# xindonglin99/allsteps_isaaclab

Measured on AMD Instinct MI355X. Metric: env-steps/sec (whole node), Allsteps-v0 at 4096 envs, 1/2/4/8 MI355X, higher is better.
Workload: dtype f32; 1 GPU; Allsteps-v0 biped walker, 4096 envs/GPU, stone curriculum level 0, decimation 4 x dt 1/240; num_envs_per_gpu=4096, global_envs=4096, parallelism=dp1 (env shards, no collective in step)

## Files before the change

allsteps_isaaclab_amd/csrc/allsteps_kernels.hip:

```cpp
#include <hip/hip_runtime.h>

#include "../../include/allsteps.h"
#include "allsteps_device.h"
#include "allsteps_kernels.h"

#include "step_scratch.h"
#include "step_lanes.h"
#include "step_dynamics.h"
#include "step_collide.h"
#include "step_solve.h"
#include "step_report.h"
#include "step_task.h"

namespace as {

template <int NV, uint64_t SKIP>
__global__ __launch_bounds__(kStepThreads) __attribute__((amdgpu_waves_per_eu(2, 2))) void k_step(StepArgs P) {
  __shared__ Smem sm;
  CK* Kc = (CK*)P.consts;
  const Consts& K = *(const Consts*)Kc;
  const int el = threadIdx.x >> 5, lane = threadIdx.x & 31;
  const int n = P.n;
  EnvS& s = sm.env[el];
  const as_state_t& st = P.st;
  Stamp ts{P.stamps, sm.stamp_acc, 0ull};
  ts.start();
  int e_raw = xcd_block(blockIdx.x, gridDim.x) * EPB + el;
  if (P.wave_map) e_raw = P.wave_map[EPB * blockIdx.x + el];
  const ConstV4* rowp = (const ConstV4*)&Kc->lane[lane];
  u32x4 rc[kLaneChunks];
#pragma unroll
  for (int k = 0; k < kLaneChunks; ++k) rc[k] = rowp[k];
  const int cur = *(const __attribute__((address_space(4))) int32_t*)st.curriculum;
  const float cur_gain = Kc->task.gain_curriculum[lane < 10 ? lane : 0];
  const float cur_term = Kc->task.term_curriculum[lane < 10 ? lane : 0];
  const bool valid = e_raw < n;
  const int e = valid ? e_raw : n - 1;
  if (P.wave_map && blockIdx.x >= (gridDim.x >> 1)) __builtin_amdgcn_s_setprio(1);
  const __attribute__((address_space(4))) as_model_t& m = Kc->model;
  const int nh = m.num_hinges;
  const __attribute__((address_space(4))) as_task_t& T = Kc->task;
  const int l3 = lane < 3 ? lane : 0, l4 = lane < 4 ? lane : 0, lh = lane < nh ? lane : 0;
  const int ns3 = 3 * T.num_steps;
  const int k0 = lane < ns3 ? lane : 0, k1 = lane + G < ns3 ? lane + G : 0;
  const float v_rp = st.root_pos[l3 * n + e], v_rl = st.root_lin[l3 * n + e], v_ra = st.root_ang[l3 * n + e];
  const float v_rq = st.root_quat[l4 * n + e];
  const float v_q = st.q[lh * n + e], v_qd = st.qd[lh * n + e];
  const float* actp = P.mode != kModeReset ? P.actions : st.q;
// ... 49 lines not shown
  if (lane < 4) s.root_quat[lane] = v_rq;
  if (lane == 0) { s.ndrop = 0; s.nrows = 0; }
  if (lane < nh) {
    int i = (int)rc[9].w - 1;
    s.qi[i] = v_q;
    s.u[6 + i] = v_qd;
    float a = fminf(fmaxf(v_a, -1.f), 1.f);
    s.act[lane] = a;
    s.tau[i] = gain * row_gear * a;
    s.qt[i] = Kc->act.action_scale * a + row_dq;
    if (P.cmd) {
      s.tau[i] = v_c;
      s.qt[i] = v_c;
    }
  }
  if (lane < ns3) s.stones[lane] = v_s0;
  if (lane + G < ns3) s.stones[lane + G] = v_s1;
  if (lane < kPkWords) s.pk[lane] = v_pk;
  __syncthreads();
  ts.mark(kStLoad);
  const bool do_physics = P.mode == kModeStep || P.mode == kModePhysics;
  if (do_physics) {
    const int substeps = Kc->sim.substeps;
    for (int left = substeps - 1; left >= 0; --left) {
      const ReportDesc* rp = P.rep;
      asm volatile("" : "+s"(rp));
      if (rp && left == 0) report_store_qd(rp, n, Kc, s, lane, e, valid);
      substep<NV, SKIP>(K, sm, s, lane, tp, gc, lc, mask, ts);
      rp = P.rep;
      asm volatile("" : "+s"(rp));
      if (rp) report_store(rp, n, s, lane, e, valid, left);
    }
  }
  const u32x4* rowg = (const u32x4*)&K.lane[lane];
  const u32x4 rr8 = rowg[8], rr9 = rowg[9];
  const float rs_q = __uint_as_float(rr8.z), rs_qm = __uint_as_float(rr8.w), rs_sg = __uint_as_float(rr9.x);
  const float rs_lo = __uint_as_float(rr9.y), rs_hi = __uint_as_float(rr9.z);
  const int rs_li = (int)rr9.w;
  float rd_m = 0.f, rd_n = 0.f;
  if (P.reset_draws && P.mode != kModePhysics) {
    rd_m = P.reset_draws[(size_t)e * 22];
    rd_n = P.reset_draws[(size_t)e * 22 + 1 + lh];
  }
  asm volatile("" ::: "memory");
  if (do_physics) {
    fk<false>(*Kc, s, lane, tp, lc, Kc->max_path);
    if (lane == 0) { s.mask[0] = mask[0]; s.mask[1] = mask[1]; s.mask[2] = mask[2]; s.mask[3] = mask[3]; }
  }
  ts.mark(kStFKFinal);
  if (lane == 0 && !do_physics) { s.mask[0] = mask[0]; s.mask[1] = mask[1]; }
  __syncthreads();
  float bp[9];
  if (do_physics) {
    const int ls[3] = {m.torso_link, m.foot_link[0], m.foot_link[1]};
    for (int b = 0; b < 3; ++b)
      for (int k = 0; k < 3; ++k) bp[3 * b + k] = s.root_pos[k] + s.p[ls[b]][k];
  } else {
    for (int k = 0; k < 9; ++k) bp[k] = __uint_as_float(s.pk[kPkBody + k]);
  }
  int idx = (int)s.pk[kPkIdx], prev = (int)s.pk[kPkPrev], next = (int)s.pk[kPkNext], count = (int)s.pk[kPkCount];
  int swing = (int)s.pk[kPkSwing], ep_len = (int)s.pk[kPkEpLen];
  float pot = __uint_as_float(s.pk[kPkPot]), old_pot = __uint_as_float(s.pk[kPkOldPot]);
  float fc[2] = {__uint_as_float(s.pk[kPkFc0]), __uint_as_float(s.pk[kPkFc1])};
  uint32_t episode = s.pk[kPkEpisode];
  bool done = false;
  Useful u{};
  if (P.mode == kModeStep || P.mode == kModeTask) {
    ep_len += 1;
    compute_useful(T, s.root_pos, s.root_quat, bp, s.stones, 1, s.mask[0], s.mask[1], idx, prev, next, count,
                   swing, pot, old_pot, fc, true, u);
    float a2 = 0.f, en = 0.f;
    int atlim = 0;
    if (lane < nh) {
      const int li = rs_li;
      float a = s.act[lane];
      a2 = a * a;
      en = fabsf(s.u[6 + li - 1] * a);
      atlim = fabsf(scale_transform(s.qi[li - 1], rs_lo, rs_hi)) > 0.99f;
    }
    a2 = half_sum(a2);
    en = half_sum(en);
    uint64_t bl = __ballot(atlim != 0);
    int nlim = __popcll(bl >> (32 * el) & 0xffffffffull);
    const float* lv = s.u;
    float speed = sqrtf(lv[0] * lv[0] + lv[1] * lv[1] + lv[2] * lv[2]);
    bool time_out = ep_len >= T.max_episode_length - 1;
    bool fell = u.h < term_h;
    bool so_fast = speed > 5.0f;
    bool died = s.root_pos[2] < T.fall_abs;
    bool terminated = fell || so_fast || died;
// ... 1 lines not shown
    bool roll_v = (u.roll > 0.4f) || (u.roll < -0.4f);
    bool pitch_v = (u.pitch > 0.4f) || (u.pitch < -0.2f);
    float roll_cost = roll_v ? fabsf(u.roll) : 0.f;
    float pitch_cost = pitch_v ? fabsf(u.pitch) : 0.f;
    float speed_cost = speed > 1.6f ? speed - 1.6f : 0.f;
    float action_cost = T.action * sqrtf(a2);
    float energy_cost = T.energy * en;
    float limit_cost = (float)nlim * T.joint_limit;
    bool cond = u.reached && count == 1 && idx < T.num_steps - 1;
    float step_rew = cond ? 50.0f * as_expf(-u.dist_s / 0.25f) : 0.f;
    bool bonus_c = idx == T.num_steps - 1 && u.body_dist < 0.15f;
    float total = T.alive + progress;
    total = total - roll_cost;
    total = total - pitch_cost;
    total = total - speed_cost;
    total = total - energy_cost;
    total = total - action_cost;
    total = total - limit_cost;
    total = total + step_rew;
    total = total + (bonus_c ? 10.0f : 0.f);
    float rew = terminated ? T.death : total;
    done = terminated || time_out;
    if (valid && lane == 0) {
      P.reward[e] = rew;
      P.terminated[e] = terminated ? 1 : 0;
      P.truncated[e] = time_out ? 1 : 0;
    }
  } else if (P.mode == kModeReset) {
    done = P.reset_mask == nullptr || P.reset_mask[e] != 0;
  }
  if (P.mode != kModePhysics) {
    const int cidx = valid ? idx : 0;
    const bool vdone = valid && done;
    const int wsum = __builtin_amdgcn_readlane(cidx, 0) + __builtin_amdgcn_readlane(cidx, 32);
    const bool wdone = __any(vdone);
    const int ndr = valid ? s.ndrop : 0;
    const int wdrop = __builtin_amdgcn_readlane(ndr, 0) + __builtin_amdgcn_readlane(ndr, 32);
    if (threadIdx.x == 0) {
      atomicAdd(&P.counters[kCntStride * (1 + (int)(blockIdx.x % kCntSlots))], wsum);
      if (wdrop) atomicAdd(&P.counters[kCntDropped], wdrop);
      if (wdone) P.counters[0] = 1;
      if (T.regen_footsteps) P.counters[kCntLevel] = cur;
    }
  }
  ts.mark(kStTask);
  const bool any_done = __any(done);
  const bool regen = T.regen_footsteps && P.mode != kModePhysics && done && idx > T.num_steps / 2;
  if (P.mode != kModePhysics && any_done) {
    if (done) {
      float dm = rd_m, dn = rd_n;
      if (!P.reset_draws) {
        float blk[4];
        philox_block(P.seed, (uint32_t)(P.env_offset + e), episode, 0u, kResetTag, blk);
        dm = blk[0];
        if (lane < nh) {
          const int k = 1 + lane;
          philox_block(P.seed, (uint32_t)(P.env_offset + e), episode, (uint32_t)(k >> 2), kResetTag, blk);
          const int sl = k & 3;
          dn = sl == 0 ? blk[0] : (sl == 1 ? blk[1] : (sl == 2 ? blk[2] : blk[3]));
        }
      }
      ep_len = 0;
      old_pot = 0.f; pot = 0.f; count = 0; swing = 0; idx = 1; prev = 0; next = 2;
      const bool mirror = dm > 0.5f;
      if (mirror) swing ^= 1;
      if (lane < nh) {
        const float sign = mirror ? rs_sg : 1.f;
        float jp = mirror ? rs_qm : rs_q;
        float jv = 0.f * sign;
        int li = rs_li;
        float x = jp + (dn * (T.noise_hi - T.noise_lo) + T.noise_lo);
        float sc = fminf(fmaxf(scale_transform(x, rs_lo, rs_hi), T.clip_lo), T.clip_hi);
        s.qi[li - 1] = unscale_transform(sc, rs_lo, rs_hi);
        s.u[6 + li - 1] = jv;
      }
      if (lane < 3) {
        const float ir[3] = {T.init_root[0], T.init_root[1], T.init_root[2]};
        s.root_pos[lane] = lane == 0 ? ir[0] : (lane == 1 ? ir[1] : ir[2]);
        s.u[lane] = 0.f;
        s.u[3 + lane] = 0.f;
      }
      if (lane == 0) {
        float sg = mirror ? -1.f : 1.f;
        s.root_quat[0] = 1.f;
        s.root_quat[1] = 0.f * sg;
        s.root_quat[2] = 0.f * sg;
        s.root_quat[3] = 0.f * sg;
      }
      episode += 1u;
    }
    __syncthreads();
    fk<false>(*Kc, s, lane, tp, lc, Kc->max_path);
    if (done) {
      const int ls[3] = {m.torso_link, m.foot_link[0], m.foot_link[1]};
      for (int b = 0; b < 3; ++b)
        for (int k = 0; k < 3; ++k) bp[3 * b + k] = s.root_pos[k] + s.p[ls[b]][k];
    }
  }
  __syncthreads();
  if (P.obs) {
    int i2 = idx, p2 = prev, n2 = next, c2 = count, w2 = swing;
    float pot2 = pot, op2 = old_pot, fc2[2] = {fc[0], fc[1]};
    Useful u2 = u;
    compute_useful(T, s.root_pos, s.root_quat, bp, s.stones, 1, s.mask[0], s.mask[1], i2, p2, n2, c2, w2, pot2,
                   op2, fc2, true, u2, any_done || !(P.mode == kModeStep || P.mode == kModeTask));
    float* ob = s.x.obs;
    uint32_t* side = P.side;
    if (lane == 0) {
      ob[0] = u2.h;
      ob[1] = u2.roll;
      ob[2] = u2.pitch;
      float vb[3];
      quat_rotate_inverse(s.root_quat, s.u, vb);
      ob[3] = vb[0]; ob[4] = vb[1]; ob[5] = vb[2];
      ob[48] = fc2[0];
      ob[49] = fc2[1];
    }
    if (lane < nh) {
      const int li = rs_li;
      ob[6 + lane] = scale_transform(s.qi[li - 1], rs_lo, rs_hi);
      ob[27 + lane] = fminf(fmaxf(s.u[6 + li - 1] * T.dof_vel_scale, -5.f), 5.f);
    }
    if (lane < 6) {
      const int t = lane < 3 ? lane : lane - 3;
      const int ti = lane < 3 ? (t == 0 ? p2 : (t == 1 ? i2 : n2)) : (t == 0 ? prev : (t == 1 ? idx : next));
      const float tw[3] = {s.stones[3 * ti], s.stones[3 * ti + 1], s.stones[3 * ti + 2]};
      float o3[3];
      subtract_frame_transforms(s.root_pos, s.root_quat, tw, o3);
      if (lane < 3) {
        for (int k = 0; k < 3; ++k) ob[50 + 3 * t + k] = o3[k];
      } else if (valid) {
        for (int k = 0; k < 3; ++k) side[(kSideState + 2 + 3 * t + k) * n + e] = __float_as_uint(o3[k]);
      }
    }
    __syncthreads();
    if (valid) {
      float* orow = P.obs + (size_t)e * AS_OBS_DIM;
      orow[lane] = ob[lane];
      if (lane < AS_OBS_DIM - 32) orow[32 + lane] = ob[32 + lane];
      if (lane == 0) {
        const uint32_t sv[kSideState + 2] = {(uint32_t)idx, (uint32_t)prev, (uint32_t)next, (uint32_t)count,
                                             (uint32_t)swing, __float_as_uint(pot), __float_as_uint(old_pot),
                                             __float_as_uint(fc[0]), __float_as_uint(fc[1]),
                                             __float_as_uint(fc[0]), __float_as_uint(fc[1])};
        for (int k = 0; k < kSideState + 2; ++k) side[k * n + e] = sv[k];
        side[kSideRegen * n + e] = regen ? 1u : 0u;
      }
    }
    idx = i2; prev = p2; next = n2; count = c2; swing = w2;
    pot = pot2; old_pot = op2; fc[0] = fc2[0]; fc[1] = fc2[1];
  }
  ts.mark(kStReset);
  if (valid) {
    if (lane < 3) {
      st.root_pos[lane * n + e] = s.root_pos[lane];
      st.root_lin[lane * n + e] = s.u[lane];
      st.root_ang[lane * n + e] = s.u[3 + lane];
    }
    if (lane < 4) st.root_quat[lane * n + e] = s.root_quat[lane];
    if (lane < nh) {
      int i = rs_li - 1;
      st.q[lane * n + e] = s.qi[i];
      st.qd[lane * n + e] = s.u[6 + i];
    }
    if (lane < 9) {
      float v = bp[0];
#pragma unroll
      for (int k = 1; k < 9; ++k) v = (lane == k) ? bp[k] : v;
      st.body_pos[lane * n + e] = v;
    }
    if (lane == 0) {
      P.side[kSideCost * n + e] = done ? 0u : (uint32_t)s.nrows;
      st.contact_mask[e] = s.mask[0];
      st.contact_mask[n + e] = s.mask[1];
      if (st.contact_mask_hind) {
        st.contact_mask_hind[e] = s.mask[2];
        st.contact_mask_hind[n + e] = s.mask[3];
      }
      if (P.mode != kModePhysics) {
        st.idx[e] = idx; st.prev[e] = prev; st.next[e] = next; st.count[e] = count; st.swing[e] = swing;
        st.ep_len[e] = ep_len; st.pot[e] = pot; st.old_pot[e] = old_pot;
        st.foot_contact[e] = fc[0]; st.foot_contact[n + e] = fc[1];
        st.episode[e] = episode;
      }
    }
  }
  ts.mark(kStStore);
  ts.flush();
}

}

#include "task_kernels.h"
#include "body_state_kernel.h"
#include "contact_forces_kernel.h"
#include "noise_kernels.h"
#include "event_kernels.h"
#include "contact_timer_kernels.h"
#include "ray_caster_kernels.h"
#include "imu_kernels.h"
#include "frame_transformer_kernels.h"
#include "ray_camera_kernels.h"
#include "command_kernels.h"
#include "observation_kernels.h"
#include "reward_kernels.h"
#include "termination_kernels.h"
#include "action_kernels.h"

namespace as {


bool step_supported_nv(int nv) { return nv == 27 || nv == 18; }

hipError_t launch_step(const StepArgs& a, int nv, bool sweep_skip, hipStream_t stream) {
  int blocks = (a.n + EPB - 1) / EPB;
  if (nv == 27 && sweep_skip)
    hipLaunchKernelGGL((k_step<27, kSweepSkip27>), dim3(blocks), dim3(kStepThreads), 0, stream, a);
  else if (nv == 27)
    hipLaunchKernelGGL((k_step<27, 0ull>), dim3(blocks), dim3(kStepThreads), 0, stream, a);
  else if (nv == 18 && sweep_skip)
    hipLaunchKernelGGL((k_step<18, kSweepSkip18>), dim3(blocks), dim3(kStepThreads), 0, stream, a);
  else if (nv == 18)
    hipLaunchKernelGGL((k_step<18, 0ull>), dim3(blocks), dim3(kStepThreads), 0, stream, a);
  else
    return hipErrorInvalidValue;
  return hipGetLastError();
}

hipError_t launch_obs(const ObsArgs& a, hipStream_t stream) {
  int blocks = (a.n + 63) / 64;
  hipLaunchKernelGGL(k_obs, dim3(blocks), dim3(64), 0, stream, a);
  return hipGetLastError();
}

hipError_t launch_stones(const StonesArgs& a, hipStream_t stream) {
  int blocks = (a.n + 255) / 256;
  hipLaunchKernelGGL(k_stones, dim3(blocks), dim3(256), 0, stream, a);
  return hipGetLastError();
}

hipError_t launch_quad(const QuadArgs& a, hipStream_t stream) {
  hipLaunchKernelGGL(k_quad<false>, dim3((a.n + kQuadEnvs - 1) / kQuadEnvs), dim3(4 * kQuadEnvs), 0, stream, a,
                     (const uint8_t*)nullptr);
  return hipGetLastError();
}

// ... 148 lines not shown
```

allsteps_isaaclab_amd/csrc/step_collide.h:

```cpp
#pragma once

#include <hip/hip_runtime.h>

#include "allsteps_pair_group.h"
#include "step_lanes.h"
#include "step_scratch.h"

namespace as {


__device__ void emit_contact(EnvS& s, int slot, int ncap, int link, int link2, int stone, int foot, const float* P,
                             const float* n, float sep, float r) {
  if (slot >= ncap) return;
  s.clink[slot] = link; s.clink2[slot] = link2; s.cstone[slot] = stone; s.cfoot[slot] = foot; s.csep[slot] = sep;
  for (int k = 0; k < 3; ++k) { s.cn[slot][k] = n[k]; s.cpt[slot][k] = P[k] - n[k] * r; }
}

struct GeomC {
  int link, type, foot;
  float r, p0[3], p1[3];
  uint32_t anc;
};
__device__ __forceinline__ float capsule_contact_sel(const float* a1, const float* b1, float r1, const float* a2,
                                                     const float* b2, float r2, float* P, float* n) {
// ... 16 lines not shown
  const float sq = as_clamp01((hi ? b - c : -c) / a);
  const float s = pa ? 0.f : (pe || lo || hi) ? sq : sm;
  const float t = pa ? (pe ? 0.f : as_clamp01(tq)) : pe ? 0.f : lo ? 0.f : hi ? 1.f : tq;
  float c1[3], c2[3], w[3];
#pragma unroll
  for (int k = 0; k < 3; ++k) {
    c1[k] = fmaf(s, d1[k], a1[k]);
    c2[k] = fmaf(t, d2[k], a2[k]);
    w[k] = c1[k] - c2[k];
  }
  const float dist = sqrtf(as_dot3(w, w));
  const bool nz = dist > 1e-9f;
  const float inv = 1.0f / dist;
  n[0] = nz ? w[0] * inv : 0.f;
  n[1] = nz ? w[1] * inv : 0.f;
  n[2] = nz ? w[2] * inv : 1.f;
  const float sep = dist - r1 - r2;
  const float off = fmaf(0.5f, sep, r2);
#pragma unroll
  for (int k = 0; k < 3; ++k) P[k] = fmaf(off, n[k], c2[k]);
  return sep;
}

__device__ __forceinline__ int collide(const Consts& K, EnvS& s, int lane, int ncap, const GeomC& gc, const float* h,
                                       float margin, int gcap, Stamp& ts) {
  const as_model_t& m = K.model;
  const int nst = K.task.num_steps, ng = m.num_geoms, npri = m.num_priority_geoms, nsp = m.num_self_pairs;
  constexpr int kSelfW = AS_MAX_SELF_PAIRS / G;
  int spw[kSelfW];
#pragma unroll
  for (int i = 0; i < kSelfW; ++i) spw[i] = G * i + lane < nsp ? m.self_pair[G * i + lane] : 0;
  const bool gv = lane < ng;
  const int link = gc.link, gtype = gc.type, foot = gc.foot;
  const float r = gc.r;
  float a[3], bb[3];
  {
    float t0[3], t1[3];
    matvec3(s.R[link], gc.p0, t0);
    matvec3(s.R[link], gc.p1, t1);
    for (int k = 0; k < 3; ++k) { a[k] = s.p[link][k] + t0[k]; bb[k] = s.p[link][k] + t1[k]; }
  }
  const float L = sqrtf((bb[0] - a[0]) * (bb[0] - a[0]) + (bb[1] - a[1]) * (bb[1] - a[1]) +
                        (bb[2] - a[2]) * (bb[2] - a[2]));
  const float mid[3] = {0.5f * (a[0] + bb[0]), 0.5f * (a[1] + bb[1]), 0.5f * (a[2] + bb[2])};
  float blo[3], bhi[3], ext[6];
#pragma unroll
  for (int k = 0; k < 3; ++k) {
    const float e = gtype == 0 ? a[k] : fminf(a[k], bb[k]);
// ... 275 lines not shown
```

allsteps_isaaclab_amd/csrc/step_dynamics.h:

```cpp
#pragma once

#include <hip/hip_runtime.h>

#include "step_lanes.h"
#include "step_scratch.h"

namespace as {

struct LinkC {
  float oq[4], ax[3], an[3], op[3];
};
__device__ __forceinline__ LinkC load_link(const Consts& K, int lane) {
  const as_model_t& m = K.model;
  const int i = lane >= 1 && lane < m.num_links ? lane : 0;
  LinkC c;
#pragma unroll
  for (int k = 0; k < 4; ++k) c.oq[k] = m.offset_quat[i][k];
#pragma unroll
  for (int k = 0; k < 3; ++k) {
    c.ax[k] = m.axis[i][k];
    c.an[k] = m.anchor[i][k];
    c.op[k] = m.offset_pos[i][k];
  }
  return c;
// ... 79 lines not shown
      B[4] = Iw[0] + mass * (cc - c[0] * c[0]);
      B[5] = Iw[4] + mass * (cc - c[1] * c[1]);
      B[6] = Iw[8] + mass * (cc - c[2] * c[2]);
      B[7] = Iw[1] - mass * c[0] * c[1];
      B[8] = Iw[2] - mass * c[0] * c[2];
      B[9] = Iw[5] - mass * c[1] * c[2];
      if (i > 0) {
        float a[3], o[3];
        matvec3(R, lc.ax, a);
        matvec3(R, lc.an, o);
        for (int k = 0; k < 3; ++k) o[k] += p[k];
        float S[6] = {a[0], a[1], a[2], 0.f, 0.f, 0.f};
        cross3(o, a, S + 3);
        const float qd = s.u[6 + i - 1];
        *reinterpret_cast<v4f*>(&s.S[6 + i - 1][0]) = v4f{S[0], S[1], S[2], S[3]};
        *reinterpret_cast<v4f*>(&s.S[6 + i - 1][4]) = v4f{S[4], S[5], 0.f, 0.f};
#pragma unroll
        for (int k = 0; k < 6; ++k) d.Sq[i][k] = S[k] * qd;
      }
    }
  }
  if constexpr (kDyn) {
    if (lane == kZeroRow) {
#pragma unroll
      for (int k = 0; k < 10; ++k) d.Ib[kZeroRow][k] = 0.f;
#pragma unroll
      for (int k = 0; k < 6; ++k) d.Sq[kZeroRow][k] = 0.f;
    }
  }
  if constexpr (kDyn) {
    float c0[3];
    matvec3(R0, m.com[0], c0);
    if (lane < 3) s.c0[lane] = c0[lane];
    if (lane < 6) {
      float S[6] = {0.f, 0.f, 0.f, 0.f, 0.f, 0.f};
      const int k = lane % 3;
      if (lane < 3) {
        S[3 + k] = 1.f;
      } else {
        float e[3] = {0.f, 0.f, 0.f};
        e[k] = 1.f;
        S[k] = 1.f;
        cross3(c0, e, S + 3);
      }
      *reinterpret_cast<v4f*>(&s.S[lane][0]) = v4f{S[0], S[1], S[2], S[3]};
      *reinterpret_cast<v4f*>(&s.S[lane][4]) = v4f{S[4], S[5], 0.f, 0.f};
    }
  }
  __syncthreads();
}
// ... 20 lines not shown
    const float* u = s.u;
    float wxc[3], vxw[3];
    cross3(s.c0, u + 3, wxc);
    cross3(u, u + 3, vxw);
    for (int k = 0; k < 3; ++k) {
      V[k] = u[3 + k];
      V[3 + k] = u[k] + wxc[k];
      A[k] = 0.f;
      A[3 + k] = vxw[k];
    }
  }
  if (lane < nl) {
    path_sum<6, 4>(tp.lpath & ~1u, max_path, V, d.Sq);
    if (lane > 0) {
      float Sq[6], cr[6];
#pragma unroll
      for (int k = 0; k < 6; ++k) Sq[k] = d.Sq[lane][k];
      crm(V, Sq, cr);
#pragma unroll
      for (int k = 0; k < 6; ++k) d.b.cr[lane][k] = cr[k];
    }
  }
  if (lane == kZeroRow) {
#pragma unroll
    for (int k = 0; k < 6; ++k) d.b.cr[kZeroRow][k] = 0.f;
  }
  __syncthreads();
  float f[6], Ib[10];
  if (lane < nl) {
    path_sum<6, 4>(tp.lpath & ~1u, max_path, A, d.b.cr);
#pragma unroll
    for (int k = 0; k < 10; ++k) Ib[k] = d.Ib[lane][k];
    float IA[6], IV[6], x[6];
    inertia_mul(Ib, A, IA);
    inertia_mul(Ib, V, IV);
    crf(V, IV, x);
    const float mg[3] = {0.f, 0.f, Ib[0] * gravity};
    float cxmg[3];
    cross3(d.c[lane], mg, cxmg);
    for (int k = 0; k < 3; ++k) {
      f[k] = IA[k] + x[k] - cxmg[k];
      f[3 + k] = IA[3 + k] + x[3 + k] - mg[k];
    }
  }
  if (lane < LMAX) {
    const bool lv = lane < nl;
#pragma unroll
    for (int k = 0; k < 6; ++k) d.xt[k][lane & 1][lane >> 1] = lv ? f[k] : 0.f;
// ... 251 lines not shown
```

allsteps_isaaclab_amd/csrc/step_lanes.h:

```cpp
#pragma once

#include <hip/hip_runtime.h>

#include "step_scratch.h"

namespace as {


template <int CTRL>
__device__ __forceinline__ float dpp(float v) {
  return __int_as_float(__builtin_amdgcn_update_dpp(0, __float_as_int(v), CTRL, 0xF, 0xF, true));
}

__device__ __forceinline__ float readlane_f(float v, int l) { return __int_as_float(__builtin_amdgcn_readlane(__float_as_int(v), l)); }

__device__ __forceinline__ float row_pair_sum(float v) {
  const auto p = __builtin_amdgcn_permlane16_swap(__float_as_int(v), __float_as_int(v), false, false);
  return __int_as_float(p[0]) + __int_as_float(p[1]);
}

__device__ __forceinline__ float half_sum(float v) {
  v += dpp<0xB1>(v);
  v += dpp<0x4E>(v);
  v += dpp<0x141>(v);
// ... 65 lines not shown
#pragma unroll
  for (int p = 0; p < P; ++p) {
    const auto s = __builtin_amdgcn_permlane16_swap(__float_as_int(v[2 * p]), __float_as_int(v[2 * p + 1]), false, false);
    c[p] = fminf(__int_as_float(s[0]), __int_as_float(s[1]));
  }
#pragma unroll
  for (int p = 0; p < P; ++p) c[p] = fminf(c[p], dpp<0xB1>(c[p]));
#pragma unroll
  for (int p = 0; p < P; ++p) c[p] = fminf(c[p], dpp<0x4E>(c[p]));
#pragma unroll
  for (int p = 0; p < P; ++p) c[p] = fminf(c[p], dpp<0x141>(c[p]));
#pragma unroll
  for (int p = 0; p < P; ++p) c[p] = fminf(c[p], dpp<0x140>(c[p]));
#pragma unroll
  for (int p = 0; p < P; ++p) {
    const auto s = __builtin_amdgcn_permlane16_swap(__float_as_int(c[p]), __float_as_int(c[p]), false, false);
    v[2 * p] = __int_as_float(s[0]);
    v[2 * p + 1] = __int_as_float(s[1]);
  }
}

constexpr int kWaveRecFlag = 31, kWaveRecBase = 64, kWaveRecWords = 30;
static_assert(16 + kNumStamps <= kWaveRecFlag && kNumStamps + 14 <= kWaveRecWords, "stamp slots");
struct Stamp {
  unsigned long long* p;
  unsigned long long* acc;
  unsigned long long t;
  unsigned long long t0 = 0ull, rt0 = 0ull;
  unsigned rows = 0u, cons = 0u, prs = 0u, lvls = 0u;
  __device__ void start() {
    if (p) {
      if (threadIdx.x < kNumStamps) acc[threadIdx.x] = 0ull;
      t = t0 = __builtin_amdgcn_s_memtime();
      rt0 = __builtin_amdgcn_s_memrealtime();
      __syncthreads();
    }
  }
  __device__ void count(int nrow, int nc) {
    if (p) {
      rows += (unsigned)nrow;
      cons += (unsigned)nc;
    }
  }
  __device__ void pairs(int np, int level) {
    if (p) {
      const unsigned mx = prs >> 16 > (unsigned)np ? prs >> 16 : (unsigned)np;
      prs = ((prs + (unsigned)np) & 0xffffu) | (mx << 16);
// ... 76 lines not shown
```

allsteps_isaaclab_amd/csrc/step_scratch.h:

```cpp
#pragma once

#include <hip/hip_runtime.h>

#include "../../include/allsteps.h"
#include "allsteps_device.h"
#include "allsteps_kernels.h"

namespace as {

constexpr int G = 32;
constexpr int EPB = 2;
constexpr int LMAX = kMaxLinks;
constexpr int NVMAX = 6 + LMAX - 1;
constexpr int MAXC = AS_MAX_CONTACTS;
constexpr int MAXR = AS_MAX_ROWS;
constexpr int NST = AS_NUM_STONES;
constexpr int kBisectIters = 12;
constexpr int kPairsPerChunk = G;
static_assert(kPairsPerChunk - 1 + G <= 64, "pending pair list (PhaseScratch::col.pl)");
typedef float v4f __attribute__((ext_vector_type(4)));
typedef float v2f __attribute__((ext_vector_type(2)));

static_assert(NVMAX <= G, "one lane per generalized velocity");
static_assert(LMAX <= G, "one lane per link");
// ... 79 lines not shown
  int rlink[MAXR];
  float rsign[MAXR];
  float cpt[MAXC][3], cn[MAXC][3], csep[MAXC];
  int clink[MAXC], clink2[MAXC], cstone[MAXC], cfoot[MAXC];
  float u[NVMAX];
  float qi[LMAX];
  float tau[LMAX];
  float qt[LMAX];
  float act[AS_ACT_DIM];
  float stones[NST * 3];
  float root_pos[3], root_quat[4];
  int cand[NST];
  uint32_t mask[4];
  int ndrop;
  int nrows;
  uint32_t pk[20];
};
enum { kPkIdx = 0, kPkPrev, kPkNext, kPkCount, kPkSwing, kPkEpLen, kPkPot, kPkOldPot, kPkFc0, kPkFc1, kPkEpisode,
       kPkBody, kPkWords = kPkBody + 9 };

struct Smem {
  EnvS env[EPB];
  Topo topo[G];
  unsigned long long stamp_acc[kNumStamps];
  int maxrow;
};

}
```

allsteps_isaaclab_amd/csrc/step_solve.h:

```cpp
#pragma once

#include <hip/hip_runtime.h>

#include "step_collide.h"
#include "step_dynamics.h"
#include "step_lanes.h"
#include "step_scratch.h"

namespace as {

__device__ void tangents(const float* n, float* t1, float* t2) {
  float e[3] = {1.f, 0.f, 0.f};
  if (fabsf(n[0]) > 0.9f) { e[0] = 0.f; e[1] = 1.f; }
  cross3(n, e, t1);
  float inv = 1.0f / sqrtf(dot3(t1, t1));
  for (int k = 0; k < 3; ++k) t1[k] *= inv;
  cross3(n, t1, t2);
}

template <int NC>
__device__ __forceinline__ void contact_flag(const EnvS& s, int lane, int nce, float dt, uint32_t (&b)[4]) {
  static_assert(NC <= MAXC, "contacts");
  const int cl = lane < MAXC ? lane : 0;
  const int f = s.cfoot[cl], st = s.cstone[cl];
// ... 109 lines not shown
      float t1 = fmaf(-vg[1], m1.x, fmaf(m1.y, m1.x, lamr[r + 1]));
      float t2 = fmaf(-vg[2], m2.x, fmaf(m2.y, m2.x, lamr[r + 2]));
      const float mu_g = m1.z, off_g = m2.z;
      const float l0 = __builtin_amdgcn_fmed3f(fmaf(-vg[0], m0.x, fmaf(m0.y, m0.x, lamr[r])), 0.f, __builtin_inff());
      const float d0 = l0 - lamr[r];
      lamr[r] = l0;
      const float blo = fmaf(-mu_g, l0, 0.f), bhi = fmaf(mu_g, l0, off_g);
      t1 = fmaf(-k10, d0, t1);
      t2 = fmaf(-k20, d0, t2);
      uj = fmaf(Wc[r], d0, uj);
      const float l1 = __builtin_amdgcn_fmed3f(t1, blo, bhi);
      const float d1 = l1 - lamr[r + 1];
      lamr[r + 1] = l1;
      t2 = fmaf(-k21, d1, t2);
      uj = fmaf(Wc[r + 1], d1, uj);
      const float l2 = __builtin_amdgcn_fmed3f(t2, blo, bhi);
      const float d2 = l2 - lamr[r + 2];
      lamr[r + 2] = l2;
      uj = fmaf(Wc[r + 2], d2, uj);
    }
  }
}

template <int NV, uint64_t SKIP>
__device__ void substep(const Consts& K0, Smem& sm, EnvS& s, int lane0, const Topo& tp0, const GeomC& gc,
                        const LinkC& lc, uint32_t (&mask_out)[4], Stamp& ts) {
  CK* kp = (CK*)(&K0);
  int lane = lane0;
  asm volatile("" : "+s"(kp), "+v"(lane));
  const Consts& K = *(const Consts*)(kp);
  const Topo& tp = tp0;
  const as_model_t& m = K.model;
  const float dt = K.sim.dt;
  const int nh = m.num_hinges;
  int smp = K.max_path;
  asm volatile("" : "+s"(smp));
  if (K.act.mode == AS_ACT_DC_MOTOR && lane < nh) {
    const as_actuator_t& A = K.act;
    s.tau[lane] = as_dc_motor(s.qt[lane], s.qi[lane], s.u[6 + lane], A.stiffness, A.damping, A.saturation_effort,
                              A.effort_limit, A.velocity_limit);
  }
  fk<true>(K, s, lane, tp, lc, smp);
  ts.mark(kStFK);
  float Sj[6], Fj[6];
  dynamics<NV>(K, s, lane, tp, K.sim.gravity, Sj, Fj, smp);
  ts.mark(kStLinkQ);
  typedef SweepLayout<NV> SL;
  constexpr int NP = SL::NP;
  float Hr[NP];
  h_row<NV>(s, lane, tp, gc.anc, Sj, Fj, *reinterpret_cast<float(*)[NV]>(Hr));
  ts.mark(kStDyn);
  {
    float Hs[NP];
#pragma unroll
    for (int k = 0; k < NV; ++k) Hs[SL::pos(SL::padded(k))] = Hr[k];
#pragma unroll
    for (int q = 0; q < NP - NV; ++q) Hs[SL::pos(SL::PAD + q)] = lane == NV + q ? 1.f : 0.f;
    sweep_inverse<NV, SKIP>(s, lane, Hs);
#pragma unroll
    for (int k = 0; k < NV; ++k) Hr[k] = lane < NV ? -Hs[SL::pos(SL::padded(k))] : 0.f;
#pragma unroll
    for (int k = NV; k < NP; ++k) Hr[k] = 0.f;
  }
  ts.mark(kStChol);
  float uj = 0.f;
  {
    float acc = 0.f;
#pragma unroll
    for (int k = 0; k < NV; ++k) acc = fmaf(Hr[k], s.b[k], acc);
    if (lane < NV) {
      uj = fmaf(dt, acc, s.u[lane]);
      s.u[lane] = uj;
    }
  }
  __syncthreads();
  ts.mark(kStSolve);
  int lo_v = 0, hi_v = 0;
  float err_lo = 0.f, err_hi = 0.f;
  if (lane < nh) {
    float qv = s.qi[lane], pred = qv + dt * s.u[6 + lane];
    err_lo = tp.lo - qv;
    err_hi = qv - tp.hi;
    lo_v = pred < tp.lo;
    hi_v = pred > tp.hi;
  }
  int ltotal;
  const int lpos = half_scan3(lo_v + hi_v, ltotal);
// ... 95 lines not shown
          const float jc1 = __uint_as_float(jb & (0u - ((pm1 >> lnk) & 1u)));
          const float jc2 = __uint_as_float(jb & (0u - ((pm2 >> lnk) & 1u)));
          const uint32_t jl = __float_as_uint(sg) & (-1 - lk == j ? ~0u : 0u);
          jq[e] = __uint_as_float(((__float_as_uint(jc1 - jc2)) | jl) & live);
        } else {
          jq[e] = 0.f;
        }
      }
      Jr[2 * q] = v2f{jq[0], jq[1]};
      Jr[2 * q + 1] = v2f{jq[2], jq[3]};
      if (lane < MAXR) *reinterpret_cast<v4f*>(&s.x.k.Jm[lane][4 * q]) = v4f{jq[0], jq[1], jq[2], jq[3]};
    }
    const uint32_t pm = pm1 | pm2;
    uint32_t dm = ((pm & 1u) ? 0x3Fu : 0u) | ((pm >> 1) << 6);
    if (!con && lane < MAXR) dm = 1u << ((-1 - lk) & 31);
    dm = lane < nrow ? dm : 0u;
    uint32_t dd = 0u;
    half_or2(dm, dd);
    jmask = (uint32_t)__builtin_amdgcn_readlane((int)dm, 0) | (uint32_t)__builtin_amdgcn_readlane((int)dm, 32);
  }
  __syncthreads();
  ts.mark(kStRows);
  float Wc[MAXR], Jc[MAXR];
  w_rows<NV>(s, lane, nrow, Hr, Jr, Jc, Wc, jmask);
  __syncthreads();
  ts.mark(kStWsolve);
  const int iters = K.sim.pgs_iters;
  float lamr[MAXR];
#pragma unroll
  for (int r = 0; r < MAXR; ++r) lamr[r] = 0.f;
  static_assert(MAXR / kRowGroup == 10, "group-count dispatch");
  switch ((__builtin_amdgcn_readfirstlane(maxrow) + kRowGroup - 1) / kRowGroup) {
    case 1: pgs_sweeps<1>(s, iters, uj, lamr, Jc, Wc); break;
    case 2: pgs_sweeps<2>(s, iters, uj, lamr, Jc, Wc); break;
    case 3: pgs_sweeps<3>(s, iters, uj, lamr, Jc, Wc); break;
    case 4: pgs_sweeps<4>(s, iters, uj, lamr, Jc, Wc); break;
    case 5: pgs_sweeps<5>(s, iters, uj, lamr, Jc, Wc); break;
    case 6: pgs_sweeps<6>(s, iters, uj, lamr, Jc, Wc); break;
    case 7: pgs_sweeps<7>(s, iters, uj, lamr, Jc, Wc); break;
    case 8: pgs_sweeps<8>(s, iters, uj, lamr, Jc, Wc); break;
    case 9: pgs_sweeps<9>(s, iters, uj, lamr, Jc, Wc); break;
    case 10: pgs_sweeps<10>(s, iters, uj, lamr, Jc, Wc); break;
    default: break;
  }
  const int nce = min(nc, (nrow + kRowGroup - 1) / kRowGroup);
  if (lane < NV) s.u[lane] = uj;
  if (lane < MAXC) {
    float ln = 0.f;
#pragma unroll
    for (int c = 0; c < MAXC; ++c) ln = lane == c ? lamr[3 * c] : ln;
    ln = 3 * lane < nrow ? ln : 0.f;
    const int key = lane < nce ? ((s.cfoot[lane] + 1) << 8) | (s.cstone[lane] + 1) : -1;
    *reinterpret_cast<v4f*>(s.x.cf[lane]) =
        v4f{ln * s.cn[lane][0], ln * s.cn[lane][1], ln * s.cn[lane][2], __int_as_float(key)};
  }
  __syncthreads();
  ts.mark(kStPGS);
  {
    uint32_t b[4] = {0u, 0u, 0u, 0u};
    contact_flag<MAXC>(s, lane, nce, dt, b);
    half_or2(b[0], b[1]);
    half_or2(b[2], b[3]);
#pragma unroll
    for (int k = 0; k < 4; ++k) mask_out[k] = b[k];
  }
  float rq[4], rp[3];
  {
    const float* u = s.u;
    float c0w[3];
    for (int k = 0; k < 3; ++k) c0w[k] = fmaf(dt, u[k], s.root_pos[k] + s.c0[k]);
    const float* w = u + 3;
    const float wn = sqrtf(dot3(w, w));
    const float th = wn * dt;
    float sn, cs;
    as_sincosf(0.5f * th, &sn, &cs);
    const float sc = sn / wn;
    const bool big = th > 1e-12f;
    const float dq[4] = {big ? cs : 1.f, big ? w[0] * sc : 0.5f * dt * w[0], big ? w[1] * sc : 0.5f * dt * w[1],
                         big ? w[2] * sc : 0.5f * dt * w[2]};
    const float* q0 = s.root_quat;
    float nq[4] = {dq[0] * q0[0] - dq[1] * q0[1] - dq[2] * q0[2] - dq[3] * q0[3],
                   dq[0] * q0[1] + dq[1] * q0[0] + dq[2] * q0[3] - dq[3] * q0[2],
                   dq[0] * q0[2] - dq[1] * q0[3] + dq[2] * q0[0] + dq[3] * q0[1],
                   dq[0] * q0[3] + dq[1] * q0[2] - dq[2] * q0[1] + dq[3] * q0[0]};
    const float qn = 1.0f / sqrtf(nq[0] * nq[0] + nq[1] * nq[1] + nq[2] * nq[2] + nq[3] * nq[3]);
    for (int k = 0; k < 4; ++k) rq[k] = nq[k] * qn;
    float Rn[9], cl[3];
    quat_to_mat(rq, Rn);
    matvec3(Rn, m.com[0], cl);
    for (int k = 0; k < 3; ++k) rp[k] = c0w[k] - cl[k];
  }
  if (lane < nh) {
    float v = fminf(fmaxf(s.u[6 + lane], -K.sim.max_joint_vel), K.sim.max_joint_vel);
    s.u[6 + lane] = v;
    s.qi[lane] = fmaf(dt, v, s.qi[lane]);
  }
  if (lane == 0) {
    for (int k = 0; k < 4; ++k) s.root_quat[k] = rq[k];
    for (int k = 0; k < 3; ++k) s.root_pos[k] = rp[k];
  }
  __syncthreads();
  ts.mark(kStIntegrate);
}

}
```

Before: 35.40 million env-steps/s.

## Split diagnostic stamp kernel and rematerialize constants to cut live registers

Adds a compile-time Stamp<false> no-op variant and a separate k_step_diag kernel, so the default kernel carries no timing stamps or stamp LDS array. Kernel arguments after the substep loop and sim constants inside the substep are re-read through opaque pointers (kernarg segment, constant address space), and asm barriers are placed on lane and zero values. This is meant to shorten live ranges and lower SGPR/VGPR pressure and LDS use. In exchange it adds extra scalar loads and relies on the compiler following these register hints.

```diff
diff --git a/allsteps_isaaclab_amd/csrc/allsteps_kernels.hip b/allsteps_isaaclab_amd/csrc/allsteps_kernels.hip
--- a/allsteps_isaaclab_amd/csrc/allsteps_kernels.hip
+++ b/allsteps_isaaclab_amd/csrc/allsteps_kernels.hip
@@ -14,16 +14,36 @@
 
 namespace as {
 
-template <int NV, uint64_t SKIP>
-__global__ __launch_bounds__(kStepThreads) __attribute__((amdgpu_waves_per_eu(2, 2))) void k_step(StepArgs P) {
-  __shared__ Smem sm;
-  CK* Kc = (CK*)P.consts;
+typedef const __attribute__((address_space(4))) StepArgs KArgs;
+
+template <bool kDiag>
+struct StepLds {
+  Smem sm;
+};
+template <>
+struct StepLds<true> {
+  Smem sm;
+  unsigned long long stamp_acc[kNumStamps];
+};
+
+template <int NV, uint64_t SKIP, bool kDiag>
+__device__ __forceinline__ void step_body(const StepArgs& P, KArgs* kargs) {
+  __shared__ StepLds<kDiag> lds;
+  Smem& sm = lds.sm;
+  KArgs* ka = kargs;
+  asm volatile("" : "+s"(ka));
+  CK* Kc = (CK*)ka->consts;
   const Consts& K = *(const Consts*)Kc;
   const int el = threadIdx.x >> 5, lane = threadIdx.x & 31;
-  const int n = P.n;
+  const int n = ka->n;
   EnvS& s = sm.env[el];
   const as_state_t& st = P.st;
-  Stamp ts{P.stamps, sm.stamp_acc, 0ull};
+  Stamp<kDiag> ts;
+  if constexpr (kDiag) {
+    ts.p = P.stamps;
+    ts.acc = lds.stamp_acc;
+    ts.t = 0ull;
+  }
   ts.start();
   int e_raw = xcd_block(blockIdx.x, gridDim.x) * EPB + el;
   if (P.wave_map) e_raw = P.wave_map[EPB * blockIdx.x + el];
@@ -119,25 +139,30 @@
   const bool do_physics = P.mode == kModeStep || P.mode == kModePhysics;
   if (do_physics) {
     const int substeps = Kc->sim.substeps;
+    const ReportDesc* rep = ka->rep;
     for (int left = substeps - 1; left >= 0; --left) {
-      const ReportDesc* rp = P.rep;
+      const ReportDesc* rp = rep;
       asm volatile("" : "+s"(rp));
       if (rp && left == 0) report_store_qd(rp, n, Kc, s, lane, e, valid);
       substep<NV, SKIP>(K, sm, s, lane, tp, gc, lc, mask, ts);
-      rp = P.rep;
+      rp = rep;
       asm volatile("" : "+s"(rp));
       if (rp) report_store(rp, n, s, lane, e, valid, left);
     }
   }
+  KArgs* qa = kargs;
+  asm volatile("" : "+s"(qa));
+  KArgs& Q = *qa;
+  const __attribute__((address_space(4))) as_state_t& sq = Q.st;
   const u32x4* rowg = (const u32x4*)&K.lane[lane];
   const u32x4 rr8 = rowg[8], rr9 = rowg[9];
   const float rs_q = __uint_as_float(rr8.z), rs_qm = __uint_as_float(rr8.w), rs_sg = __uint_as_float(rr9.x);
   const float rs_lo = __uint_as_float(rr9.y), rs_hi = __uint_as_float(rr9.z);
   const int rs_li = (int)rr9.w;
   float rd_m = 0.f, rd_n = 0.f;
-  if (P.reset_draws && P.mode != kModePhysics) {
-    rd_m = P.reset_draws[(size_t)e * 22];
-    rd_n = P.reset_draws[(size_t)e * 22 + 1 + lh];
+  if (Q.reset_draws && Q.mode != kModePhysics) {
+    rd_m = Q.reset_draws[(size_t)e * 22];
+    rd_n = Q.reset_draws[(size_t)e * 22 + 1 + lh];
   }
   asm volatile("" ::: "memory");
   if (do_physics) {
@@ -162,7 +187,7 @@
   uint32_t episode = s.pk[kPkEpisode];
   bool done = false;
   Useful u{};
-  if (P.mode == kModeStep || P.mode == kModeTask) {
+  if (Q.mode == kModeStep || Q.mode == kModeTask) {
     ep_len += 1;
     compute_useful(T, s.root_pos, s.root_quat, bp, s.stones, 1, s.mask[0], s.mask[1], idx, prev, next, count,
                    swing, pot, old_pot, fc, true, u);
@@ -210,14 +235,14 @@
     float rew = terminated ? T.death : total;
     done = terminated || time_out;
     if (valid && lane == 0) {
-      P.reward[e] = rew;
-      P.terminated[e] = terminated ? 1 : 0;
-      P.truncated[e] = time_out ? 1 : 0;
-    }
-  } else if (P.mode == kModeReset) {
-    done = P.reset_mask == nullptr || P.reset_mask[e] != 0;
-  }
-  if (P.mode != kModePhysics) {
+      Q.reward[e] = rew;
+      Q.terminated[e] = terminated ? 1 : 0;
+      Q.truncated[e] = time_out ? 1 : 0;
+    }
+  } else if (Q.mode == kModeReset) {
+    done = Q.reset_mask == nullptr || Q.reset_mask[e] != 0;
+  }
+  if (Q.mode != kModePhysics) {
     const int cidx = valid ? idx : 0;
     const bool vdone = valid && done;
     const int wsum = __builtin_amdgcn_readlane(cidx, 0) + __builtin_amdgcn_readlane(cidx, 32);
@@ -225,25 +250,25 @@
     const int ndr = valid ? s.ndrop : 0;
     const int wdrop = __builtin_amdgcn_readlane(ndr, 0) + __builtin_amdgcn_readlane(ndr, 32);
     if (threadIdx.x == 0) {
-      atomicAdd(&P.counters[kCntStride * (1 + (int)(blockIdx.x % kCntSlots))], wsum);
-      if (wdrop) atomicAdd(&P.counters[kCntDropped], wdrop);
-      if (wdone) P.counters[0] = 1;
-      if (T.regen_footsteps) P.counters[kCntLevel] = cur;
+      atomicAdd(&Q.counters[kCntStride * (1 + (int)(blockIdx.x % kCntSlots))], wsum);
+      if (wdrop) atomicAdd(&Q.counters[kCntDropped], wdrop);
+      if (wdone) Q.counters[0] = 1;
+      if (T.regen_footsteps) Q.counters[kCntLevel] = cur;
     }
   }
   ts.mark(kStTask);
   const bool any_done = __any(done);
-  const bool regen = T.regen_footsteps && P.mode != kModePhysics && done && idx > T.num_steps / 2;
-  if (P.mode != kModePhysics && any_done) {
+  const bool regen = T.regen_footsteps && Q.mode != kModePhysics && done && idx > T.num_steps / 2;
+  if (Q.mode != kModePhysics && any_done) {
     if (done) {
       float dm = rd_m, dn = rd_n;
-      if (!P.reset_draws) {
+      if (!Q.reset_draws) {
         float blk[4];
-        philox_block(P.seed, (uint32_t)(P.env_offset + e), episode, 0u, kResetTag, blk);
+        philox_block(Q.seed, (uint32_t)(Q.env_offset + e), episode, 0u, kResetTag, blk);
         dm = blk[0];
         if (lane < nh) {
           const int k = 1 + lane;
-          philox_block(P.seed, (uint32_t)(P.env_offset + e), episode, (uint32_t)(k >> 2), kResetTag, blk);
+          philox_block(Q.seed, (uint32_t)(Q.env_offset + e), episode, (uint32_t)(k >> 2), kResetTag, blk);
           const int sl = k & 3;
           dn = sl == 0 ? blk[0] : (sl == 1 ? blk[1] : (sl == 2 ? blk[2] : blk[3]));
         }
@@ -286,14 +311,14 @@
     }
   }
   __syncthreads();
-  if (P.obs) {
+  if (Q.obs) {
     int i2 = idx, p2 = prev, n2 = next, c2 = count, w2 = swing;
     float pot2 = pot, op2 = old_pot, fc2[2] = {fc[0], fc[1]};
     Useful u2 = u;
     compute_useful(T, s.root_pos, s.root_quat, bp, s.stones, 1, s.mask[0], s.mask[1], i2, p2, n2, c2, w2, pot2,
-                   op2, fc2, true, u2, any_done || !(P.mode == kModeStep || P.mode == kModeTask));
+                   op2, fc2, true, u2, any_done || !(Q.mode == kModeStep || Q.mode == kModeTask));
     float* ob = s.x.obs;
-    uint32_t* side = P.side;
+    uint32_t* side = Q.side;
     if (lane == 0) {
       ob[0] = u2.h;
       ob[1] = u2.roll;
@@ -323,7 +348,7 @@
     }
     __syncthreads();
     if (valid) {
-      float* orow = P.obs + (size_t)e * AS_OBS_DIM;
+      float* orow = Q.obs + (size_t)e * AS_OBS_DIM;
       orow[lane] = ob[lane];
       if (lane < AS_OBS_DIM - 32) orow[32 + lane] = ob[32 + lane];
       if (lane == 0) {
@@ -341,40 +366,52 @@
   ts.mark(kStReset);
   if (valid) {
     if (lane < 3) {
-      st.root_pos[lane * n + e] = s.root_pos[lane];
-      st.root_lin[lane * n + e] = s.u[lane];
-      st.root_ang[lane * n + e] = s.u[3 + lane];
-    }
-    if (lane < 4) st.root_quat[lane * n + e] = s.root_quat[lane];
+      sq.root_pos[lane * n + e] = s.root_pos[lane];
+      sq.root_lin[lane * n + e] = s.u[lane];
+      sq.root_ang[lane * n + e] = s.u[3 + lane];
+    }
+    if (lane < 4) sq.root_quat[lane * n + e] = s.root_quat[lane];
     if (lane < nh) {
       int i = rs_li - 1;
-      st.q[lane * n + e] = s.qi[i];
-      st.qd[lane * n + e] = s.u[6 + i];
+      sq.q[lane * n + e] = s.qi[i];
+      sq.qd[lane * n + e] = s.u[6 + i];
     }
     if (lane < 9) {
       float v = bp[0];
 #pragma unroll
       for (int k = 1; k < 9; ++k) v = (lane == k) ? bp[k] : v;
-      st.body_pos[lane * n + e] = v;
+      sq.body_pos[lane * n + e] = v;
     }
     if (lane == 0) {
-      P.side[kSideCost * n + e] = done ? 0u : (uint32_t)s.nrows;
-      st.contact_mask[e] = s.mask[0];
-      st.contact_mask[n + e] = s.mask[1];
-      if (st.contact_mask_hind) {
-        st.contact_mask_hind[e] = s.mask[2];
-        st.contact_mask_hind[n + e] = s.mask[3];
-      }
-      if (P.mode != kModePhysics) {
-        st.idx[e] = idx; st.prev[e] = prev; st.next[e] = next; st.count[e] = count; st.swing[e] = swing;
-        st.ep_len[e] = ep_len; st.pot[e] = pot; st.old_pot[e] = old_pot;
-        st.foot_contact[e] = fc[0]; st.foot_contact[n + e] = fc[1];
-        st.episode[e] = episode;
+      Q.side[kSideCost * n + e] = done ? 0u : (uint32_t)s.nrows;
+      sq.contact_mask[e] = s.mask[0];
+      sq.contact_mask[n + e] = s.mask[1];
+      if (sq.contact_mask_hind) {
+        sq.contact_mask_hind[e] = s.mask[2];
+        sq.contact_mask_hind[n + e] = s.mask[3];
+      }
+      if (Q.mode != kModePhysics) {
+        sq.idx[e] = idx; sq.prev[e] = prev; sq.next[e] = next; sq.count[e] = count; sq.swing[e] = swing;
+        sq.ep_len[e] = ep_len; sq.pot[e] = pot; sq.old_pot[e] = old_pot;
+        sq.foot_contact[e] = fc[0]; sq.foot_contact[n + e] = fc[1];
+        sq.episode[e] = episode;
       }
     }
   }
   ts.mark(kStStore);
   ts.flush();
+}
+
+__device__ __forceinline__ KArgs* step_kargs() { return (KArgs*)__builtin_amdgcn_kernarg_segment_ptr(); }
+
+template <int NV, uint64_t SKIP>
+__global__ __launch_bounds__(kStepThreads) __attribute__((amdgpu_waves_per_eu(2, 2))) void k_step(StepArgs P) {
+  step_body<NV, SKIP, false>(P, step_kargs());
+}
+
+template <int NV, uint64_t SKIP>
+__global__ __launch_bounds__(kStepThreads) __attribute__((amdgpu_waves_per_eu(2, 2))) void k_step_diag(StepArgs P) {
+  step_body<NV, SKIP, true>(P, step_kargs());
 }
 
 }
@@ -400,16 +437,24 @@
 
 bool step_supported_nv(int nv) { return nv == 27 || nv == 18; }
 
+template <int NV, uint64_t SKIP>
+static void launch_step_twin(const StepArgs& a, hipStream_t stream) {
+  const int blocks = (a.n + EPB - 1) / EPB;
+  if (a.stamps)
+    hipLaunchKernelGGL((k_step_diag<NV, SKIP>), dim3(blocks), dim3(kStepThreads), 0, stream, a);
+  else
+    hipLaunchKernelGGL((k_step<NV, SKIP>), dim3(blocks), dim3(kStepThreads), 0, stream, a);
+}
+
 hipError_t launch_step(const StepArgs& a, int nv, bool sweep_skip, hipStream_t stream) {
-  int blocks = (a.n + EPB - 1) / EPB;
   if (nv == 27 && sweep_skip)
-    hipLaunchKernelGGL((k_step<27, kSweepSkip27>), dim3(blocks), dim3(kStepThreads), 0, stream, a);
+    launch_step_twin<27, kSweepSkip27>(a, stream);
   else if (nv == 27)
-    hipLaunchKernelGGL((k_step<27, 0ull>), dim3(blocks), dim3(kStepThreads), 0, stream, a);
+    launch_step_twin<27, 0ull>(a, stream);
   else if (nv == 18 && sweep_skip)
-    hipLaunchKernelGGL((k_step<18, kSweepSkip18>), dim3(blocks), dim3(kStepThreads), 0, stream, a);
+    launch_step_twin<18, kSweepSkip18>(a, stream);
   else if (nv == 18)
-    hipLaunchKernelGGL((k_step<18, 0ull>), dim3(blocks), dim3(kStepThreads), 0, stream, a);
+    launch_step_twin<18, 0ull>(a, stream);
   else
     return hipErrorInvalidValue;
   return hipGetLastError();
diff --git a/allsteps_isaaclab_amd/csrc/step_collide.h b/allsteps_isaaclab_amd/csrc/step_collide.h
--- a/allsteps_isaaclab_amd/csrc/step_collide.h
+++ b/allsteps_isaaclab_amd/csrc/step_collide.h
@@ -62,8 +62,9 @@
   return sep;
 }
 
+template <class TS>
 __device__ __forceinline__ int collide(const Consts& K, EnvS& s, int lane, int ncap, const GeomC& gc, const float* h,
-                                       float margin, int gcap, Stamp& ts) {
+                                       float margin, int gcap, TS& ts) {
   const as_model_t& m = K.model;
   const int nst = K.task.num_steps, ng = m.num_geoms, npri = m.num_priority_geoms, nsp = m.num_self_pairs;
   constexpr int kSelfW = AS_MAX_SELF_PAIRS / G;
diff --git a/allsteps_isaaclab_amd/csrc/step_dynamics.h b/allsteps_isaaclab_amd/csrc/step_dynamics.h
--- a/allsteps_isaaclab_amd/csrc/step_dynamics.h
+++ b/allsteps_isaaclab_amd/csrc/step_dynamics.h
@@ -125,10 +125,12 @@
   }
   if constexpr (kDyn) {
     if (lane == kZeroRow) {
-#pragma unroll
-      for (int k = 0; k < 10; ++k) d.Ib[kZeroRow][k] = 0.f;
-#pragma unroll
-      for (int k = 0; k < 6; ++k) d.Sq[kZeroRow][k] = 0.f;
+      float z = 0.f;
+      asm volatile("" : "+v"(z));
+#pragma unroll
+      for (int k = 0; k < 10; ++k) d.Ib[kZeroRow][k] = z;
+#pragma unroll
+      for (int k = 0; k < 6; ++k) d.Sq[kZeroRow][k] = z;
     }
   }
   if constexpr (kDyn) {
@@ -195,8 +197,10 @@
     }
   }
   if (lane == kZeroRow) {
-#pragma unroll
-    for (int k = 0; k < 6; ++k) d.b.cr[kZeroRow][k] = 0.f;
+    float z = 0.f;
+    asm volatile("" : "+v"(z));
+#pragma unroll
+    for (int k = 0; k < 6; ++k) d.b.cr[kZeroRow][k] = z;
   }
   __syncthreads();
   float f[6], Ib[10];
diff --git a/allsteps_isaaclab_amd/csrc/step_lanes.h b/allsteps_isaaclab_amd/csrc/step_lanes.h
--- a/allsteps_isaaclab_amd/csrc/step_lanes.h
+++ b/allsteps_isaaclab_amd/csrc/step_lanes.h
@@ -111,7 +111,18 @@
 
 constexpr int kWaveRecFlag = 31, kWaveRecBase = 64, kWaveRecWords = 30;
 static_assert(16 + kNumStamps <= kWaveRecFlag && kNumStamps + 14 <= kWaveRecWords, "stamp slots");
-struct Stamp {
+template <bool kOn>
+struct Stamp;
+template <>
+struct Stamp<false> {
+  __device__ __forceinline__ void start() {}
+  __device__ __forceinline__ void count(int, int) {}
+  __device__ __forceinline__ void pairs(int, int) {}
+  __device__ __forceinline__ void mark(int) {}
+  __device__ __forceinline__ void flush() {}
+};
+template <>
+struct Stamp<true> {
   unsigned long long* p;
   unsigned long long* acc;
   unsigned long long t;
diff --git a/allsteps_isaaclab_amd/csrc/step_scratch.h b/allsteps_isaaclab_amd/csrc/step_scratch.h
--- a/allsteps_isaaclab_amd/csrc/step_scratch.h
+++ b/allsteps_isaaclab_amd/csrc/step_scratch.h
@@ -125,8 +125,6 @@
 struct Smem {
   EnvS env[EPB];
   Topo topo[G];
-  unsigned long long stamp_acc[kNumStamps];
-  int maxrow;
 };
 
 }
diff --git a/allsteps_isaaclab_amd/csrc/step_solve.h b/allsteps_isaaclab_amd/csrc/step_solve.h
--- a/allsteps_isaaclab_amd/csrc/step_solve.h
+++ b/allsteps_isaaclab_amd/csrc/step_solve.h
@@ -155,17 +155,21 @@
   }
 }
 
-template <int NV, uint64_t SKIP>
+template <int NV, uint64_t SKIP, class TS>
 __device__ void substep(const Consts& K0, Smem& sm, EnvS& s, int lane0, const Topo& tp0, const GeomC& gc,
-                        const LinkC& lc, uint32_t (&mask_out)[4], Stamp& ts) {
+                        const LinkC& lc, uint32_t (&mask_out)[4], TS& ts) {
   CK* kp = (CK*)(&K0);
   int lane = lane0;
   asm volatile("" : "+s"(kp), "+v"(lane));
   const Consts& K = *(const Consts*)(kp);
   const Topo& tp = tp0;
   const as_model_t& m = K.model;
-  const float dt = K.sim.dt;
   const int nh = m.num_hinges;
+  auto fresh = [kp]() -> const Consts& {
+    CK* q = kp;
+    asm volatile("" : "+s"(q));
+    return *(const Consts*)(q);
+  };
   int smp = K.max_path;
   asm volatile("" : "+s"(smp));
   if (K.act.mode == AS_ACT_DC_MOTOR && lane < nh) {
@@ -183,6 +187,7 @@
   float Hr[NP];
   h_row<NV>(s, lane, tp, gc.anc, Sj, Fj, *reinterpret_cast<float(*)[NV]>(Hr));
   ts.mark(kStDyn);
+  const float dt = fresh().sim.dt;
   {
     float Hs[NP];
 #pragma unroll
@@ -196,6 +201,7 @@
     for (int k = NV; k < NP; ++k) Hr[k] = 0.f;
   }
   ts.mark(kStChol);
+  asm volatile("" : "+v"(lane));
   float uj = 0.f;
   {
     float acc = 0.f;
@@ -337,10 +343,15 @@
   __syncthreads();
   ts.mark(kStRows);
   float Wc[MAXR], Jc[MAXR];
+  asm volatile("" : "+v"(lane));
   w_rows<NV>(s, lane, nrow, Hr, Jr, Jc, Wc, jmask);
   __syncthreads();
   ts.mark(kStWsolve);
-  const int iters = K.sim.pgs_iters;
+  const Consts& Ki = fresh();
+  const int iters = Ki.sim.pgs_iters;
+  const float dti = Ki.sim.dt, mjv = Ki.sim.max_joint_vel;
+  const int nhi = Ki.model.num_hinges;
+  const float com0[3] = {Ki.model.com[0][0], Ki.model.com[0][1], Ki.model.com[0][2]};
   float lamr[MAXR];
 #pragma unroll
   for (int r = 0; r < MAXR; ++r) lamr[r] = 0.f;
@@ -371,9 +382,10 @@
   }
   __syncthreads();
   ts.mark(kStPGS);
+  asm volatile("" : "+v"(lane));
   {
     uint32_t b[4] = {0u, 0u, 0u, 0u};
-    contact_flag<MAXC>(s, lane, nce, dt, b);
+    contact_flag<MAXC>(s, lane, nce, dti, b);
     half_or2(b[0], b[1]);
     half_or2(b[2], b[3]);
 #pragma unroll
@@ -383,16 +395,16 @@
   {
     const float* u = s.u;
     float c0w[3];
-    for (int k = 0; k < 3; ++k) c0w[k] = fmaf(dt, u[k], s.root_pos[k] + s.c0[k]);
+    for (int k = 0; k < 3; ++k) c0w[k] = fmaf(dti, u[k], s.root_pos[k] + s.c0[k]);
     const float* w = u + 3;
     const float wn = sqrtf(dot3(w, w));
-    const float th = wn * dt;
+    const float th = wn * dti;
     float sn, cs;
     as_sincosf(0.5f * th, &sn, &cs);
     const float sc = sn / wn;
     const bool big = th > 1e-12f;
-    const float dq[4] = {big ? cs : 1.f, big ? w[0] * sc : 0.5f * dt * w[0], big ? w[1] * sc : 0.5f * dt * w[1],
-                         big ? w[2] * sc : 0.5f * dt * w[2]};
+    const float dq[4] = {big ? cs : 1.f, big ? w[0] * sc : 0.5f * dti * w[0], big ? w[1] * sc : 0.5f * dti * w[1],
+                         big ? w[2] * sc : 0.5f * dti * w[2]};
     const float* q0 = s.root_quat;
     float nq[4] = {dq[0] * q0[0] - dq[1] * q0[1] - dq[2] * q0[2] - dq[3] * q0[3],
                    dq[0] * q0[1] + dq[1] * q0[0] + dq[2] * q0[3] - dq[3] * q0[2],
@@ -402,13 +414,13 @@
     for (int k = 0; k < 4; ++k) rq[k] = nq[k] * qn;
     float Rn[9], cl[3];
     quat_to_mat(rq, Rn);
-    matvec3(Rn, m.com[0], cl);
+    matvec3(Rn, com0, cl);
     for (int k = 0; k < 3; ++k) rp[k] = c0w[k] - cl[k];
   }
-  if (lane < nh) {
-    float v = fminf(fmaxf(s.u[6 + lane], -K.sim.max_joint_vel), K.sim.max_joint_vel);
+  if (lane < nhi) {
+    float v = fminf(fmaxf(s.u[6 + lane], -mjv), mjv);
     s.u[6 + lane] = v;
-    s.qi[lane] = fmaf(dt, v, s.qi[lane]);
+    s.qi[lane] = fmaf(dti, v, s.qi[lane]);
   }
   if (lane == 0) {
     for (int k = 0; k < 4; ++k) s.root_quat[k] = rq[k];
```

New measurement: 36.06 million env-steps/s (median of 6 runs). 1.9% higher.
